# kaushik87599/Melo-GAN

Hardware: AMD Instinct MI355X
Metric: piano-roll samples/sec (G+D step), batch=64 128x256 roll (higher is better)
Workload: dtype f32; 1 GPU; cfg2: 128x256 piano-roll, batch=64 per GPU, full G+D+emotion-D step (1 critic update incl. gradient penalty + 1 generator update); global_batch=64, T=256, C=128, parallelism=dp1, graph=True

## Files before the change

### include/melo_gan_hip.h

```cpp
#ifndef MELO_GAN_HIP_H
#define MELO_GAN_HIP_H

#include <stddef.h>
#include <stdint.h>

#ifdef __cplusplus
extern "C" {
#endif

typedef void* mg_stream_t;

enum { MG_ACT_NONE = 0, MG_ACT_RELU = 1, MG_ACT_LRELU = 2, MG_ACT_GELU = 3, MG_ACT_TANH = 4 };

typedef struct mg_epilogue {
    const float* bias;
    const float* scale;
    const float* shift;
    float* zout;
    int act;
    const float* gref;
    int gact;
    const float* emul;
    const float* gscale;
    int accumulate;
// ... 46 lines not shown
#define MG_CHAIN_SLOTS 6
#define MG_CHAIN_MAX_VEC 512
enum { MG_CH_LOAD = 1, MG_CH_STORE = 2, MG_CH_LAYERNORM = 3, MG_CH_LIN_FWD = 4, MG_CH_LIN_DGRAD = 5, MG_CH_SOFTMAX_CE = 6,
       MG_CH_DHEAD = 7, MG_CH_MEAN_T = 8, MG_CH_COPY = 9 };
typedef struct mg_chain_op {
    int kind;
    int a, b;
    int n0, n1;
    int act;
    int i0, i1;
    float f0;
    const float* p0; long ld0;
    const float* p1; long ld1;
    const float* p2; long ld2;
    const float* p3; long ld3;
    float* q0; long lq0;
    float* q1; long lq1;
    const int64_t* t0;
} mg_chain_op;
int mg_row_chain(const mg_chain_op* ops, int n_ops, int rows, mg_stream_t stream);
int mg_mean_scaled(const float* src, float* out, int n, float scale, mg_stream_t stream);
int mg_stamp(unsigned long long* dst, mg_stream_t stream);

size_t mg_linear_workspace_bytes(int M, int N, int K);
int mg_linear(const float* x, const float* w, float* y, int M, int K, int N, int w_sn, int w_sc,
              const mg_epilogue* epi, int perm_L, void* work, size_t work_bytes, mg_stream_t stream);
int mg_linear_route(int M, int K, int N, int w_sn, int w_sc, int perm_L, int x_aligned, int w_aligned,
                    int* kcontig, int* vec, int* ksplit);

int mg_conv1d_wino3_supported(int B, int T, int Cin, int N);
int mg_wino3_weights(const float* w, float* wt, int N, int Cin, long w_sn, long w_sc, int flip, mg_stream_t stream);
int mg_conv1d_wino3(const float* x, const float* wt, float* y, int B, int T, int Cin, int N, const mg_epilogue* epi,
                    long lds_pad, mg_stream_t stream);
#define MG_MAX_WINO_WJOBS 8
typedef struct mg_wino3_wjob {
    const float* w;
    float* wt;
    int N, Cin;
    long w_sn, w_sc;
    int flip;
} mg_wino3_wjob;
int mg_wino3_weights_multi(const mg_wino3_wjob* jobs, int n_jobs, mg_stream_t stream);

int mg_conv_tile_config(long m_rows, int N, int scatter2);
int mg_conv_plan(int B, int Tm, int Tout, int N, int Cin, int K, int stride, int scatter2, size_t work_bytes,
                 int* ksplit, int* cps);
// ... 253 lines not shown
```

### melo-gan_amd/csrc/common.h

```cpp
#pragma once
#include <hip/hip_runtime.h>
#include <stdio.h>
#include <stdarg.h>
#include <stdint.h>
#include <atomic>
#include "../../include/melo_gan_hip.h"

#define MG_OK 0
#define MG_EARG (-1)
#define MG_EUNSUP (-2)
#define MG_EWORK (-3)
#define MG_EHIP (-4)

void mg_set_error(const char* fmt, ...);

#define MG_CHECK_ARG(cond, ...)                    \
    do {                                           \
        if (!(cond)) {                             \
            mg_set_error(__VA_ARGS__);             \
            return MG_EARG;                        \
        }                                          \
    } while (0)

#define MG_CHECK_LAUNCH(name)                                                   \
    do {                                                                        \
        hipError_t e__ = hipGetLastError();                                     \
        if (e__ != hipSuccess) {                                                \
// ... 191 lines not shown

inline int mg_lds_optin(const void* kernel, std::atomic<uint64_t>& done) {
    int dev = 0;
    MG_HIP(hipGetDevice(&dev));
    const uint64_t bit = dev < 64 ? 1ull << dev : 0;
    if (done.load(std::memory_order_relaxed) & bit) return MG_OK;
    MG_HIP(hipFuncSetAttribute(kernel, hipFuncAttributeMaxDynamicSharedMemorySize, 160 * 1024));
    done.fetch_or(bit, std::memory_order_relaxed);
    return MG_OK;
}

int mg_conv_thin_dispatch(const float* x, const float* w, float* y, int B, int Tin, int Cin, int Tout, int N, int K, int stride,
                          int flip, int transposed, int w_sn, int w_sc, long xbs, long ybs, const mg_epilogue* epi,
                          hipStream_t stream);

int mg_conv_linear_perm(const float* x, const float* w, float* y, int M, int K, int N, int w_sn, const mg_epilogue* epi,
                        int perm_L, hipStream_t stream);

__device__ __forceinline__ int mg_xcd_remap(int id, int n) {
    const int q = n >> 3, r = n & 7, x = id & 7;
    return (x < r ? x * (q + 1) : r * (q + 1) + (x - r) * q) + (id >> 3);
}

static inline int mg_ilog2_ceil(int v) {
    int l = 0;
    while ((1 << l) < v) ++l;
    return l;
}
static inline long mg_cdiv(long a, long b) { return (a + b - 1) / b; }
```

### melo-gan_amd/csrc/linear_skinny.hip

```cpp
#include "common.h"
#include <stdlib.h>
#include <type_traits>

namespace {

struct LinP {
    const float* x;
    const float* w;
    float* y;
    float* part;
    int M, K, N;
    int w_sn, w_sc;
    int ksplit;
    int gx, gy;
    int kw;
    int perm_L, perm_C;
    mg_epilogue e;
};
__device__ __forceinline__ int wrow(const LinP& p, int n) { return p.perm_L ? (n % p.perm_C) * p.perm_L + n / p.perm_C : n; }

constexpr int UNR = 8;
constexpr int NW = 8;

template <bool W_KCONTIG, bool VEC>
__global__ __launch_bounds__(64 * NW) void linear_skinny_kernel(const LinP p) {
    __shared__ float tile[NW][32][33];
    const int tid = threadIdx.x, lane = tid & 63, wave = tid >> 6;
    const int i = lane & 31, h = lane >> 5;
    const int id = mg_xcd_remap((int)blockIdx.x, (int)gridDim.x);
    const int bx = id % p.gx, byz = id / p.gx, by = byz % p.gy, bz = byz / p.gy;
    const int m0 = bx * 32, n0 = by * 32;
    const int row = min(m0 + i, p.M - 1);
    const int col = wrow(p, min(n0 + i, p.N - 1));
// ... 77 lines not shown
    for (int r = 0; r < 16; ++r) tile[wave][(r & 3) + 8 * (r >> 2) + 4 * h][i] = acc[r];
    __syncthreads();
    constexpr int NV = 1024 / (64 * NW);
    float v[NV];
    int nn[NV];
    long di[NV];
    bool ok[NV];
#pragma unroll
    for (int q = 0; q < NV; ++q) {
        const int idx = tid + 64 * NW * q;
        const int rr = idx >> 5, cc = idx & 31;
        const int m = m0 + rr, n = n0 + cc;
        ok[q] = m < p.M && n < p.N;
        nn[q] = ok[q] ? wrow(p, n) : 0;
        di[q] = ok[q] ? (long)m * p.N + n : 0;
        float t = 0.f;
#pragma unroll
        for (int w = 0; w < NW; w += 2) t += tile[w][rr][cc] + tile[w + 1][rr][cc];
        v[q] = t;
    }
    if (p.ksplit > 1) {
#pragma unroll
        for (int q = 0; q < NV; ++q)
            if (ok[q]) p.part[(long)bz * p.M * p.N + di[q]] = v[q];
        return;
    }
    mg_apply_epilogue_set<NV>(p.e, v, nn, di, ok);
#pragma unroll
    for (int q = 0; q < NV; ++q) {
        if (!ok[q]) continue;
        if (p.e.accumulate) v[q] += p.y[di[q]];
        p.y[di[q]] = v[q];
    }
}

__global__ void linear_finish_kernel(const float* __restrict__ part, float* __restrict__ y, long mn, int N, int ksplit,
                                     const mg_epilogue e, int perm_L, int perm_C) {
    const long di = (long)blockIdx.x * blockDim.x + threadIdx.x;
    if (di >= mn) return;
    float v = 0.f;
    for (int z = 0; z < ksplit; ++z) v += part[(long)z * mn + di];
    int n = (int)(di % N);
    if (perm_L) n = (n % perm_C) * perm_L + n / perm_C;
    v = mg_apply_epilogue(e, v, n, di);
    if (e.accumulate) v += y[di];
    y[di] = v;
}

int plan_ksplit(int M, int N, int K) {
    const long tiles = mg_cdiv(M, 32) * mg_cdiv(N, 32);
    int ks = 1;
    while (ks < 32 && K / (NW * ks) > 128 && tiles * ks < 512) ks *= 2;
    return ks;
}

struct LinRoute {
    bool window_gemm;
    bool kcontig, vec;
    int ksplit, kw;
};
LinRoute linear_route(int M, int K, int N, int w_sn, int w_sc, int perm_L, bool x_aligned, bool w_aligned) {
    LinRoute r{};
    if (perm_L > 1 && w_sc == 1 && M >= 128 && (K & 63) == 0 && (N & 63) == 0 && mg_cdiv(M, 64) * (long)(N / 64) >= 192 &&
        x_aligned && w_aligned && (w_sn & 3) == 0 && !getenv("MG_LINEAR_SKINNY_ONLY")) {
        r.window_gemm = true;
        r.ksplit = 1;
        return r;
    }
    r.ksplit = plan_ksplit(M, N, K);
    r.kcontig = (w_sc == 1);
    const int waves = NW * r.ksplit;
    r.vec = (K % (8 * waves) == 0) && x_aligned && (!r.kcontig || (w_aligned && (w_sn & 3) == 0));
    r.kw = r.vec ? K / waves : (int)(mg_cdiv(mg_cdiv(K, waves), 8) * 8);
    return r;
}
bool al16(const void* q) { return (((uintptr_t)q) & 15) == 0; }

}

extern "C" int mg_linear_route(int M, int K, int N, int w_sn, int w_sc, int perm_L, int x_aligned, int w_aligned,
                               int* kcontig, int* vec, int* ksplit) {
    MG_CHECK_ARG(perm_L >= 0 && (perm_L == 0 || N % perm_L == 0), "mg_linear_route: perm_L must divide N");
    MG_CHECK_ARG(M > 0 && K > 0 && N > 0 && w_sn > 0 && w_sc > 0, "mg_linear_route: bad shape");
    MG_CHECK_ARG(w_sn == 1 || w_sc == 1, "mg_linear_route: one weight stride must be 1");
    const LinRoute r = linear_route(M, K, N, w_sn, w_sc, perm_L, x_aligned != 0, w_aligned != 0);
    if (kcontig) *kcontig = r.kcontig;
    if (vec) *vec = r.vec;
    if (ksplit) *ksplit = r.ksplit;
    return r.window_gemm ? 0 : 1;
}

extern "C" size_t mg_linear_workspace_bytes(int M, int N, int K) {
    const int ks = plan_ksplit(M, N, K);
    return ks > 1 ? (size_t)ks * M * N * sizeof(float) : 0;
}

extern "C" int mg_linear(const float* x, const float* w, float* y, int M, int K, int N, int w_sn, int w_sc,
                         const mg_epilogue* epi, int perm_L, void* work, size_t work_bytes, mg_stream_t stream) {
    MG_CHECK_ARG(x && w && y, "mg_linear: null tensor");
    MG_CHECK_ARG(perm_L >= 0 && (perm_L == 0 || N % perm_L == 0), "mg_linear: perm_L must divide N");
    MG_CHECK_ARG(M > 0 && K > 0 && N > 0 && w_sn > 0 && w_sc > 0, "mg_linear: bad shape");
    MG_CHECK_ARG(w_sn == 1 || w_sc == 1, "mg_linear: one weight stride must be 1");
    const LinRoute r = linear_route(M, K, N, w_sn, w_sc, perm_L, al16(x), al16(w));
    if (r.window_gemm)
        return mg_conv_linear_perm(x, w, y, M, K, N, w_sn, epi, perm_L, (hipStream_t)stream);
    LinP p{};
    p.x = x; p.w = w; p.y = y; p.M = M; p.K = K; p.N = N; p.w_sn = w_sn; p.w_sc = w_sc;
    p.e = epi ? *epi : mg_epilogue{};
    p.perm_L = perm_L > 1 ? perm_L : 0;
    p.perm_C = p.perm_L ? N / p.perm_L : 0;
    if (p.e.scale && !p.e.shift) { mg_set_error("mg_linear: scale without shift"); return MG_EARG; }
    p.ksplit = r.ksplit;
    const bool kcontig = r.kcontig, vec = r.vec;
    p.kw = r.kw;
    if (p.ksplit > 1) {
        const size_t need = (size_t)p.ksplit * M * N * sizeof(float);
        if (!work || work_bytes < need) { mg_set_error("mg_linear: workspace too small (%zu < %zu)", work_bytes, need); return MG_EWORK; }
        p.part = (float*)work;
    }
    p.gx = (int)mg_cdiv(M, 32); p.gy = (int)mg_cdiv(N, 32);
    dim3 grid((unsigned)(p.gx * p.gy * p.ksplit));
    hipStream_t st = (hipStream_t)stream;
    if (kcontig) {
        if (vec) hipLaunchKernelGGL((linear_skinny_kernel<true, true>), grid, dim3(64 * NW), 0, st, p);
        else hipLaunchKernelGGL((linear_skinny_kernel<true, false>), grid, dim3(64 * NW), 0, st, p);
    } else {
        if (vec) hipLaunchKernelGGL((linear_skinny_kernel<false, true>), grid, dim3(64 * NW), 0, st, p);
        else hipLaunchKernelGGL((linear_skinny_kernel<false, false>), grid, dim3(64 * NW), 0, st, p);
    }
    MG_CHECK_LAUNCH("linear_skinny_kernel");
    if (p.ksplit > 1) {
        const long mn = (long)M * N;
        hipLaunchKernelGGL(linear_finish_kernel, dim3((unsigned)mg_cdiv(mn, 256)), dim3(256), 0, st,
                           (const float*)work, y, mn, N, p.ksplit, p.e, p.perm_L, p.perm_C);
        MG_CHECK_LAUNCH("linear_finish_kernel");
    }
    return MG_OK;
}
```

### melo-gan_amd/csrc/wgrad_mfma.hip

```cpp
#include "common.h"
#include <stdlib.h>
#include <type_traits>

namespace {

struct WgradP {
    const float* s[2];
    const float* l[2];
    int nb[2];
    float* part;
    float* out;
    float* bias_out;
    int Ts, Tl, A, Bc;
    int tt_log2, n_ttiles;
    int bps;
    int n_bgroups;
    int nbg0;
    long slab;
    long wslab;
    int bias_from;
    int nseg_bias;
    int vec_ok;
    int lin;
    int gx, gy, gz;
};

constexpr int RT = 64;
constexpr int BA = 32, BB = 32;

typedef unsigned u32x4 __attribute__((ext_vector_type(4)));

#ifdef MG_STAMPS
__device__ long long* mg_wstamp_buf = nullptr;
// ... 153 lines not shown
#endif
    MG_STAMP(2);
    float* red = smem;
    float* out = p.part ? p.part + (long)split * p.slab : p.out;
    constexpr int KP = K > 3 ? 3 : K;
    const int nb_cols = min(32, p.Bc - b0);
#pragma unroll
    for (int k0 = 0; k0 < K; k0 += KP) {
        const int kn = (K - k0) < KP ? (K - k0) : KP;
        __syncthreads();
#pragma unroll
        for (int k = k0; k < k0 + kn; ++k)
#pragma unroll
            for (int r = 0; r < 16; ++r)
                red[((wave * KP + (k - k0)) * 32 + (r & 3) + 8 * (r >> 2) + 4 * h) * 33 + (lane & 31)] = acc[k][r];
        __syncthreads();
#pragma unroll 4
        for (int idx = tid; idx < 32 * kn * 32; idx += 256) {
            const int ar = idx / (kn * 32), j = idx - ar * (kn * 32);
            const int bc = j / kn, kk = j - bc * kn;
            const int a = a0 + ar;
            const int o = (kk * 32 + ar) * 33 + bc;
            const float v = (red[o] + red[o + KP * 32 * 33]) + (red[o + 2 * KP * 32 * 33] + red[o + 3 * KP * 32 * 33]);
            if (a < p.A && bc < nb_cols) out[((long)a * p.Bc + b0 + bc) * K + k0 + kk] = v;
        }
    }
    MG_STAMP(3);
}

constexpr int W16_SP = 48;
template <int S> struct W16LP { static constexpr int value = S == 2 ? 40 : 48; };

template <int S, int K>
__device__ __forceinline__ bool wgrad16_applies(const WgradP& p) {
    constexpr int RMAX = (RT - 1) * S + K;
    constexpr int NL4 = (RMAX * (BB / 4) + 255) / 256 + 1;
    const int TT = 1 << p.tt_log2, TB = RT >> p.tt_log2, R = (TT - 1) * S + K;
    return ((p.A & 3) == 0) && ((p.Bc & 3) == 0) && p.vec_ok && (TB * R * (BB / 4) <= 256 * NL4) && p.tt_log2 >= 4;
}

template <int S, int K>
__device__ __forceinline__ void wgrad16_body(const WgradP& p, const int bx, const int by, const int bz) {
    constexpr int PAD = (K - 1) / 2;
    constexpr int RMAX = (RT - 1) * S + K;
    constexpr int NS4 = RT * (BA / 4) / 256;
    constexpr int NL4 = (RMAX * (BB / 4) + 255) / 256 + 1;
    constexpr int SP = W16_SP, LP = W16LP<S>::value;
// ... 131 lines not shown
        for (int k = 0; k < K; ++k) read_b(0, 0, k, fr[0]);
        MG_STAMP(1);
        for (int c = 0;;) {
            chunk(std::integral_constant<int, 0>{}, c);
            if (++c >= n_chunks) break;
            chunk(std::integral_constant<int, 1>{}, c);
            if (++c >= n_chunks) break;
        }
    }
    MG_STAMP(2);

    __syncthreads();
    constexpr int PE = K * 32 + 1;
    float* red = smem;
#pragma unroll
    for (int k = 0; k < K; ++k)
#pragma unroll
        for (int r = 0; r < 4; ++r) red[(16 * wa + 4 * kq + r) * PE + (16 * wb + li) * K + k] = acc[k][r];
    __syncthreads();
    const int nb_valid = min(32, p.Bc - b0) * K;
#pragma unroll 4
    for (int idx = tid; idx < 32 * K * 32; idx += 256) {
        const int ar = idx / (K * 32), j = idx - ar * (K * 32);
        if (a0 + ar < p.A && j < nb_valid) out[((long)(a0 + ar) * p.Bc + b0) * K + j] = red[ar * PE + j];
    }
    MG_STAMP(3);
}

constexpr int LIN_BB = 128;
__device__ __forceinline__ bool wgrad_lin_applies(const WgradP& p) {
    return p.lin != 0;
}
__device__ __forceinline__ void wgrad_lin_body(const WgradP& p, const int bx, const int by, const int bz) {
    extern __shared__ __attribute__((aligned(16))) float smem[];
    constexpr int SPL = 36, LPL = 132;
    float* Ss = smem;
    float* Ls = smem + RT * SPL;
    const int tid = threadIdx.x, lane = tid & 63, wave = tid >> 6, h = lane >> 5, c = lane & 31;
    const int a0 = bx * BA, b0 = by * LIN_BB;
    const int TB = RT;
    const int g_begin = bz * p.bps, g_end = min(g_begin + p.bps, p.n_bgroups);
    f32x16 acc;
#pragma unroll
    for (int i = 0; i < 16; ++i) acc[i] = 0.f;
    for (int g = g_begin; g < g_end; ++g) {
        const int seg_id = g < p.nbg0 ? 0 : 1;
        const int bb0 = (seg_id ? g - p.nbg0 : g) * TB;
// ... 9 lines not shown
            const f32x4 v = *reinterpret_cast<const f32x4*>(Sp + (long)(ok ? r : 0) * p.A + (ok ? a0 + 4 * q : 0));
            *reinterpret_cast<f32x4*>(Ss + r * SPL + 4 * q) = ok ? v : f32x4{0.f, 0.f, 0.f, 0.f};
        }
#pragma unroll
        for (int j = 0; j < 8; ++j) {
            const int idx = tid + 256 * j, r = idx >> 5, q = idx & 31;
            const bool ok = r < rows && b0 + 4 * q < p.Bc;
            const f32x4 v = *reinterpret_cast<const f32x4*>(Lp + (long)(ok ? r : 0) * p.Bc + (ok ? b0 + 4 * q : 0));
            *reinterpret_cast<f32x4*>(Ls + r * LPL + 4 * q) = ok ? v : f32x4{0.f, 0.f, 0.f, 0.f};
        }
        __syncthreads();
#pragma unroll 8
        for (int r2 = 0; r2 < RT / 2; ++r2) {
            const int r = 2 * r2 + h;
            acc = __builtin_amdgcn_mfma_f32_32x32x2f32(Ss[r * SPL + c], Ls[r * LPL + 32 * wave + c], acc, 0, 0, 0);
        }
    }
    float* out = p.part ? p.part + (long)bz * p.slab : p.out;
    const int b = b0 + 32 * wave + c;
    if (b < p.Bc) {
#pragma unroll
        for (int i = 0; i < 16; ++i) {
            const int a = a0 + (i & 3) + 8 * (i >> 2) + 4 * h;
            if (a < p.A) out[(long)a * p.Bc + b] = acc[i];
        }
    }
}

__device__ __forceinline__ void wgrad_bias_body(const WgradP& p, const int cb, const int bz) {
    extern __shared__ __attribute__((aligned(16))) float smem[];
    f32x4* bred = reinterpret_cast<f32x4*>(smem);
    const int tid = threadIdx.x, q = tid & 7, rl = tid >> 3;
    const bool from_s = p.bias_from == 1;
    const int C = from_s ? p.A : p.Bc, T = from_s ? p.Ts : p.Tl;
    const int TB = RT >> p.tt_log2;
    const int g_begin = bz * p.bps, g_end = min(g_begin + p.bps, p.n_bgroups);
    f32x4 acc = {0.f, 0.f, 0.f, 0.f};
    const int c = cb * 32 + 4 * q;
    for (int seg = 0; seg < p.nseg_bias && seg < 2; ++seg) {
        const int gs = seg ? p.nbg0 : 0, ge = seg ? p.n_bgroups : p.nbg0;
        const int ga = max(g_begin, gs), gb = min(g_end, ge);
        if (ga >= gb) continue;
        const int b_lo = (ga - gs) * TB, b_hi = min((gb - gs) * TB, p.nb[seg]);
        const float* base = (from_s ? p.s[seg] : p.l[seg]) + (long)b_lo * T * C;
        const long rows = (long)(b_hi - b_lo) * T;
        if (c + 3 < C && (C & 3) == 0 && p.vec_ok) {
            long r = rl;
            for (; r + 32 * 7 < rows; r += 32 * 8) {
                f32x4 v[8];
#pragma unroll
                for (int u = 0; u < 8; ++u) v[u] = *reinterpret_cast<const f32x4*>(base + (r + 32 * u) * C + c);
#pragma unroll
                for (int u = 0; u < 8; ++u) acc += v[u];
            }
            for (; r < rows; r += 32) acc += *reinterpret_cast<const f32x4*>(base + r * C + c);
        } else {
            for (long r = rl; r < rows; r += 32)
#pragma unroll
                for (int e = 0; e < 4; ++e)
                    if (c + e < C) acc[e] += base[r * C + c + e];
        }
    }
    bred[tid] = acc;
    __syncthreads();
    if (tid < 32) {
        const int ch = cb * 32 + tid;
        if (ch < C) {
            float v = 0.f;
#pragma unroll 8
            for (int g = 0; g < 32; ++g) v += bred[8 * g + (tid >> 2)][tid & 3];
            if (p.part) p.part[(long)bz * p.slab + p.wslab + ch] = v;
            else p.bias_out[ch] = v;
        }
    }
}

struct WgradJobs {
    WgradP p[MG_MAX_WGRAD_JOBS];
    int first[MG_MAX_WGRAD_JOBS + 1];
    int bfirst[MG_MAX_WGRAD_JOBS + 1];
    int n;
};
template <int S, int K>
__global__ __launch_bounds__(256, 2) void wgrad_multi_kernel(const WgradJobs J) {
    const int bid = (int)blockIdx.x;
    const bool tile = bid < J.first[J.n];
    const int* first = tile ? J.first : J.bfirst;
    int j = 0;
    while (j + 1 < J.n && bid >= first[j + 1]) ++j;
    const int b = bid - first[j];
    const WgradP& p = J.p[j];
    if (tile) {
        const int gxy = p.gx * p.gy, bz = b / gxy, r = b - bz * gxy;
        if (K == 1 && wgrad_lin_applies(p)) wgrad_lin_body(p, r % p.gx, r / p.gx, bz);
        else if (wgrad16_applies<S, K>(p)) wgrad16_body<S, K>(p, r % p.gx, r / p.gx, bz);
        else wgrad_body<S, K>(p, r % p.gx, r / p.gx, bz);
    } else {
        const int ncb = ((p.bias_from == 1 ? p.A : p.Bc) + 31) >> 5;
        wgrad_bias_body(p, b % ncb, b / ncb);
    }
}

struct ReduceJobs {
    const float* part[MG_MAX_WGRAD_JOBS];
    float* out[MG_MAX_WGRAD_JOBS];
    float* bias_out[MG_MAX_WGRAD_JOBS];
    long n[MG_MAX_WGRAD_JOBS], wn[MG_MAX_WGRAD_JOBS];
    int nsplit[MG_MAX_WGRAD_JOBS];
    int first[MG_MAX_WGRAD_JOBS + 1];
    int njobs;
};
__global__ __launch_bounds__(256) void reduce_slabs_multi_kernel(const ReduceJobs J) {
    __shared__ float sh[4][64];
    int j = 0;
    while (j + 1 < J.njobs && (int)blockIdx.x >= J.first[j + 1]) ++j;
    const float* __restrict__ part = J.part[j];
    const long n = J.n[j], wn = J.wn[j];
    const int nsplit = J.nsplit[j];
    const int ex = threadIdx.x & 63, g = threadIdx.x >> 6;
    const long i = (long)((int)blockIdx.x - J.first[j]) * 64 + ex;
    float s = 0.f;
    if (i < n)
// ... 34 lines not shown
    if (want > ngroups) want = ngroups;
    if (want > MAX_SPLITS) want = MAX_SPLITS;
    if (want < 1) want = 1;
    pl.bps = (int)mg_cdiv(ngroups, want);
    pl.nsplit = (int)mg_cdiv(ngroups, pl.bps);
    return pl;
}

}

#ifdef MG_STAMPS
extern "C" int mg_dbg_set_wstamps(long long* buf) {
    return hipMemcpyToSymbol(HIP_SYMBOL(mg_wstamp_buf), &buf, sizeof(buf)) == hipSuccess ? 0 : 1;
}
#endif

extern "C" size_t mg_wgrad_workspace_bytes(int A, int Bc, int K, int nb_total, int Ts) {
    int lg = mg_ilog2_ceil(Ts);
    const int lgrt = mg_ilog2_ceil(RT);
    if (lg > lgrt) lg = lgrt;
    const int TB = RT >> lg;
    long ns = mg_cdiv(nb_total, TB) + 1;
    if (ns > MAX_SPLITS) ns = MAX_SPLITS;
    return (size_t)ns * ((size_t)A * (size_t)Bc * (size_t)K + (size_t)(A > Bc ? A : Bc)) * sizeof(float);
}

namespace {
int build_wgrad(const float* s0, const float* l0, int nb0, const float* s1, const float* l1, int nb1, float* out,
                float* bias_out, int bias_from, int Ts, int Tl, int A, int Bc, int K, int stride, void* work,
                size_t work_bytes, WgradP& p, Plan& pl, size_t& lds, dim3& grid, long want_slices = 0) {
    MG_CHECK_ARG(bias_from >= 0 && bias_from <= 2 && ((bias_from == 0) == (bias_out == nullptr)),
                 "mg_wgrad: bias_out and bias_from (1: sums of S, 2: sums of L) must be given together");
    MG_CHECK_ARG(s0 && l0 && out && nb0 > 0, "mg_wgrad: null/empty segment 0");
    MG_CHECK_ARG(nb1 == 0 || (s1 && l1), "mg_wgrad: null segment 1");
    MG_CHECK_ARG(Ts > 0 && Tl > 0 && A > 0 && Bc > 0, "mg_wgrad: bad shape");
    MG_CHECK_ARG(K == 1 || K == 3 || K == 5, "mg_wgrad: K=%d unsupported", K);
    MG_CHECK_ARG(stride == 1 || stride == 2, "mg_wgrad: stride=%d unsupported", stride);
    if (stride == 2 && K != 5) {
        mg_set_error("mg_wgrad: stride 2 needs K=5");
        return MG_EUNSUP;
    }
    pl = make_plan(A, Bc, K, nb0, nb1, Ts, want_slices);
    const long wslab = (long)A * Bc * K;
    const long slab = wslab + (bias_from == 1 ? A : bias_from == 2 ? Bc : 0);
    if (pl.nsplit > 1 && (!work || work_bytes < (size_t)pl.nsplit * slab * sizeof(float))) {
        mg_set_error("mg_wgrad: workspace too small (%zu < %zu)", work_bytes, (size_t)pl.nsplit * slab * sizeof(float));
        return MG_EWORK;
// ... 41 lines not shown
    return MG_OK;
}
}

extern "C" int mg_wgrad_multi(const mg_wgrad_job* jobs, int n_jobs, int K, int stride, void* work, size_t work_bytes,
                              mg_stream_t stream);

extern "C" int mg_wgrad(const float* s0, const float* l0, int nb0, const float* s1, const float* l1, int nb1,
                        float* out, float* bias_out, int bias_from, int Ts, int Tl, int A, int Bc, int K, int stride,
                        void* work, size_t work_bytes, mg_stream_t stream) {
    mg_wgrad_job j{};
    j.s0 = s0; j.l0 = l0; j.nb0 = nb0;
    j.s1 = s1; j.l1 = l1; j.nb1 = nb1;
    j.out = out; j.bias_out = bias_out; j.bias_from = bias_from;
    j.Ts = Ts; j.Tl = Tl; j.A = A; j.Bc = Bc;
    return mg_wgrad_multi(&j, 1, K, stride, work, work_bytes, stream);
}

extern "C" int mg_wgrad_multi(const mg_wgrad_job* jobs, int n_jobs, int K, int stride, void* work, size_t work_bytes,
                              mg_stream_t stream) {
    MG_CHECK_ARG(jobs && n_jobs > 0 && n_jobs <= MG_MAX_WGRAD_JOBS, "mg_wgrad_multi: 1..%d jobs", MG_MAX_WGRAD_JOBS);
    WgradJobs J{};
    ReduceJobs Rj{};
    size_t lds_max = 0, used = 0;
    int nblocks = 0, rblocks = 0;
    long want[MG_MAX_WGRAD_JOBS];
    {
        long target = 512;
        if (const char* f = getenv("MG_WGRAD_TARGET")) target = atol(f);
        long tiles[MG_MAX_WGRAD_JOBS], chunks[MG_MAX_WGRAD_JOBS], total = 0;
        for (int i = 0; i < n_jobs; ++i) {
            const mg_wgrad_job& q = jobs[i];
            MG_CHECK_ARG(q.A > 0 && q.Bc > 0 && q.Ts > 0 && q.Tl > 0 && q.nb0 > 0 && q.nb1 >= 0 && q.s0 && q.l0 && q.out,
                         "mg_wgrad_multi: job %d: null/empty segment 0 or bad shape", i);
            const Plan pl = make_plan(q.A, q.Bc, K, q.nb0, q.nb1, q.Ts);
            tiles[i] = mg_cdiv(q.A, BA) * mg_cdiv(q.Bc, BB);
            chunks[i] = (long)(pl.nbg0 + pl.nbg1) * pl.n_ttiles;
            total += tiles[i] * chunks[i];
        }
        long cpw = mg_cdiv(total, target);
        for (int it = 0; it < 64; ++it) {
            long wgs = 0;
            for (int i = 0; i < n_jobs; ++i) {
                const mg_wgrad_job& q = jobs[i];
                want[i] = (chunks[i] + cpw / 2) / cpw;
                if (want[i] < 1) want[i] = 1;
                const Plan pl = make_plan(q.A, q.Bc, K, q.nb0, q.nb1, q.Ts, want[i]);
                wgs += tiles[i] * pl.nsplit;
            }
            if (wgs <= target) break;
            cpw += mg_cdiv(cpw, 16);
        }
    }
    for (int i = 0; i < n_jobs; ++i) {
        const mg_wgrad_job& q = jobs[i];
        Plan pl;
        size_t lds;
        dim3 grid;
        const size_t need = mg_wgrad_workspace_bytes(q.A, q.Bc, K, q.nb0 + q.nb1, q.Ts);
        void* w = used < work_bytes && work ? (char*)work + used : nullptr;
        const int rc = build_wgrad(q.s0, q.l0, q.nb0, q.s1, q.l1, q.nb1, q.out, q.bias_out, q.bias_from, q.Ts, q.Tl, q.A,
                                   q.Bc, K, stride, w, w ? work_bytes - used : 0, J.p[i], pl, lds, grid, want[i]);
        if (rc != MG_OK) return rc;
        if (pl.nsplit > 1) {
            used += (need + 255) & ~(size_t)255;
            const int r = Rj.njobs++;
            Rj.part[r] = J.p[i].part; Rj.out[r] = q.out; Rj.bias_out[r] = q.bias_out;
            Rj.n[r] = J.p[i].slab; Rj.wn[r] = J.p[i].wslab; Rj.nsplit[r] = pl.nsplit;
            Rj.first[r] = rblocks;
            rblocks += (int)mg_cdiv(J.p[i].slab, 64);
        }
        lds_max = lds > lds_max ? lds : lds_max;
        const int ntile = J.p[i].gx * J.p[i].gy * J.p[i].gz;
        J.first[i] = nblocks;
        nblocks += ntile;
        J.bfirst[i] = (int)grid.x - ntile;
    }
    J.first[n_jobs] = nblocks;
    for (int i = 0; i < n_jobs; ++i) {
        const int nb = J.bfirst[i];
        J.bfirst[i] = nblocks;
        nblocks += nb;
    }
    J.bfirst[n_jobs] = nblocks;
    J.n = n_jobs;
    Rj.first[Rj.njobs] = rblocks;
    hipStream_t st = (hipStream_t)stream;
#define MG_WG(S_, K_) hipLaunchKernelGGL((wgrad_multi_kernel<S_, K_>), dim3((unsigned)nblocks), dim3(256), lds_max, st, J)
    if (stride == 1) {
        if (K == 1) MG_WG(1, 1); else if (K == 3) MG_WG(1, 3); else MG_WG(1, 5);
    } else {
        MG_WG(2, 5);
    }
#undef MG_WG
    MG_CHECK_LAUNCH("wgrad_multi_kernel");
    if (Rj.njobs > 0) {
        hipLaunchKernelGGL(reduce_slabs_multi_kernel, dim3((unsigned)rblocks), dim3(256), 0, st, Rj);
        MG_CHECK_LAUNCH("reduce_slabs_multi_kernel");
    }
    return MG_OK;
}
```

### melo-gan_amd/ops.py

```python
from __future__ import annotations

import ctypes as C
import functools
import math
from typing import Optional

import torch

from . import _lib as L
from ._lib import ACT_NONE, ACT_RELU, ACT_LRELU, ACT_GELU, ACT_TANH, Epilogue

Tensor = torch.Tensor


def _stream() -> C.c_void_p:
    return C.c_void_p(torch.cuda.current_stream().cuda_stream)


def _p(t: Optional[Tensor]):
    return None if t is None else C.c_void_p(t.data_ptr())


def _chk(t: Tensor, name: str, shape=None, dtype=torch.float32):
    if not isinstance(t, torch.Tensor) or not t.is_cuda:
# ... 326 lines not shown
    L.check(rc, "mg_conv16")
    return y


SKINNY_MAX_ROWS = 512


def linear_route(M: int, K: int, N: int, w_sn: int, w_sc: int, perm_L: int = 0, x_aligned: bool = True, w_aligned: bool = True):
    lib = L.load()
    kc, vec, ks = C.c_int(), C.c_int(), C.c_int()
    rc = lib.mg_linear_route(M, K, N, w_sn, w_sc, perm_L, int(x_aligned), int(w_aligned), C.byref(kc), C.byref(vec), C.byref(ks))
    if rc < 0:
        L.check(rc, "mg_linear_route")
    if rc == 0:
        return "conv_wgemm_kernel<1,1,false,true,%s>" % {22: "2,2", 12: "1,2", 11: "1,1"}[lib.mg_conv_tile_config(M, N, 0)], 1
    return "linear_skinny_kernel<%s,%s>" % ("true" if kc.value else "false", "true" if vec.value else "false"), ks.value


def _linear(x, w, y, K, N, w_sn, w_sc, epi, perm_L=0):
    M = x.shape[0]
    e = epilogue((M, N), N, **epi)
    lib = L.load()
    need = lib.mg_linear_workspace_bytes(M, N, K)
    work = workspace(need, x.device, "linear") if need else None
    sym = lambda: linear_route(M, K, N, w_sn, w_sc, perm_L, x.data_ptr() % 16 == 0, w.data_ptr() % 16 == 0)[0]
    with _observe(sym, 2.0 * M * N * K):
        rc = lib.mg_linear(_p(x), _p(w), _p(y), M, K, N, w_sn, w_sc, C.byref(e), perm_L, _p(work),
                           work.numel() if work is not None else 0, _stream())
    L.check(rc, "mg_linear")
    return y


def linear_fwd(x, w, y, perm_L: int = 0, **epi):
    _chk(x, "x")
    _chk(w, "w")
    _chk(y, "y")
    out_f, in_f = w.shape
    B = x.shape[0]
    if perm_L:
        if B > SKINNY_MAX_ROWS or out_f % perm_L or x.dim() != 2 or x.shape[1] != in_f or tuple(y.shape) != (B, perm_L, out_f // perm_L):
            raise ValueError(f"linear_fwd(perm_L={perm_L}): shape mismatch x{tuple(x.shape)} w{tuple(w.shape)} y{tuple(y.shape)}")
        return _linear(x, w, y, in_f, out_f, in_f, 1, epi, perm_L)
    if x.dim() != 2 or x.shape[1] != in_f or tuple(y.shape) != (B, out_f):
        raise ValueError(f"linear_fwd: shape mismatch x{tuple(x.shape)} w{tuple(w.shape)} y{tuple(y.shape)}")
    if B <= SKINNY_MAX_ROWS:
        return _linear(x, w, y, in_f, out_f, in_f, 1, epi)
    conv_gather(x.view(B, 1, in_f), w, y.view(B, 1, out_f), out_f, 1, 1, in_f, 1, **epi)
# ... 205 lines not shown
            _chk(ly["dw"], "dw", tuple(w.shape))
            a.dw = ly["dw"].data_ptr()
    return arr


def spectral_norm_fwd(layers, train: bool, eps: float = 1e-12):
    arr = _sn_jobs(layers, False)
    L.check(L.load().mg_spectral_norm_fwd(arr, len(layers), 1 if train else 0, float(eps), _stream()), "mg_spectral_norm_fwd")


def spectral_norm_bwd(layers):
    arr = _sn_jobs(layers, True)
    L.check(L.load().mg_spectral_norm_bwd(arr, len(layers), _stream()), "mg_spectral_norm_bwd")


def stamp(buf, i: int):
    L.check(L.load().mg_stamp(buf.data_ptr() + 8 * int(i), _stream()), "mg_stamp")


_ws_cache = {}
_ws_retired = []


def workspace(nbytes: int, device, tag: str = "default") -> Tensor:
    key = (str(device), tag, torch.cuda.current_stream().cuda_stream)
    buf = _ws_cache.get(key)
    if buf is None or buf.numel() < nbytes:
        if buf is not None:
            _ws_retired.append(buf)
        size = max(nbytes, 1 << 20, 2 * buf.numel() if buf is not None else 0)
        buf = torch.empty(size, dtype=torch.uint8, device=device)
        _ws_cache[key] = buf
    return buf


def wgrad(small: Tensor, large: Tensor, out: Tensor, K: int, stride: int,
          small2: Optional[Tensor] = None, large2: Optional[Tensor] = None, work: Optional[Tensor] = None,
          bias_out: Optional[Tensor] = None, bias_from: int = 0):
    _chk(small, "small")
    _chk(large, "large")
    _chk(out, "out")
    nb0, Ts, A = small.shape
    if large.shape[0] != nb0:
        raise ValueError("wgrad: batch mismatch")
    Tl, Bc = large.shape[1], large.shape[2]
    pad = (K - 1) // 2
    if (Tl + 2 * pad - K) // stride + 1 != Ts and not (stride == 2 and Tl == 2 * Ts):
        raise ValueError(f"wgrad: Ts={Ts} inconsistent with Tl={Tl}, K={K}, stride={stride}")
    if out.numel() != A * Bc * K:
        raise ValueError(f"wgrad: out numel {out.numel()} != {A * Bc * K}")
    nb1 = 0
    if small2 is not None:
        _chk(small2, "small2")
        _chk(large2, "large2")
        nb1 = small2.shape[0]
        if tuple(small2.shape[1:]) != (Ts, A) or tuple(large2.shape) != (nb1, Tl, Bc):
            raise ValueError("wgrad: segment 1 shape mismatch")
    if bias_out is not None:
        _chk(bias_out, "bias_out", (A if bias_from == 1 else Bc,))
        if bias_from not in (1, 2):
            raise ValueError("wgrad: bias_from must be 1 (S) or 2 (L) when bias_out is given")
    elif bias_from:
        raise ValueError("wgrad: bias_from without bias_out")
    lib = L.load()
    need = lib.mg_wgrad_workspace_bytes(A, Bc, K, nb0 + nb1, Ts)
    if work is None:
        work = workspace(need, small.device, "wgrad")
    if work.numel() * work.element_size() < need:
        raise ValueError("wgrad: workspace too small")
    with _observe(lambda: f"wgrad_multi_kernel<{stride},{K}>", 2.0 * (nb0 + nb1) * Ts * A * Bc * K):
        rc = lib.mg_wgrad(_p(small), _p(large), nb0, _p(small2), _p(large2), nb1, _p(out), _p(bias_out), bias_from,
                          Ts, Tl, A, Bc, K, stride, _p(work), work.numel() * work.element_size(), _stream())
    L.check(rc, "mg_wgrad")
    return out


def _wgrad_job(small, large, out, K, stride, small2=None, large2=None, bias_out=None, bias_from=0):
    _chk(small, "small")
    _chk(large, "large")
    _chk(out, "out")
    nb0, Ts, A = small.shape
    Tl, Bc = large.shape[1], large.shape[2]
    pad = (K - 1) // 2
    if large.shape[0] != nb0 or ((Tl + 2 * pad - K) // stride + 1 != Ts and not (stride == 2 and Tl == 2 * Ts)):
        raise ValueError(f"wgrad: S {tuple(small.shape)} inconsistent with L {tuple(large.shape)}, K={K}, stride={stride}")
    if out.numel() != A * Bc * K:
        raise ValueError(f"wgrad: out numel {out.numel()} != {A * Bc * K}")
    nb1 = 0
    if small2 is not None:
        _chk(small2, "small2")
# ... 7 lines not shown
        _chk(bias_out, "bias_out", (A if bias_from == 1 else Bc,))
    elif bias_from:
        raise ValueError("wgrad: bias_from without bias_out")
    return (small, large, nb0, small2, large2, nb1, out, bias_out, bias_from, Ts, Tl, A, Bc, K, stride)


def wgrad_multi(jobs, tag=""):
    lib = L.load()
    groups = {}
    for j in jobs:
        groups.setdefault((j[13], j[14]), []).append(j)
    for (K, stride), js in groups.items():
        for i in range(0, len(js), L.MAX_WGRAD_JOBS):
            part = js[i:i + L.MAX_WGRAD_JOBS]
            arr = (L.WgradJob * len(part))()
            need, flops = 0, 0.0
            for a, (s0, l0, nb0, s1, l1, nb1, out, bo, bf, Ts, Tl, A, Bc, _, _) in zip(arr, part):
                a.s0, a.l0, a.nb0 = s0.data_ptr(), l0.data_ptr(), nb0
                a.s1, a.l1, a.nb1 = (None if s1 is None else s1.data_ptr()), (None if l1 is None else l1.data_ptr()), nb1
                a.out, a.bias_out, a.bias_from = out.data_ptr(), (None if bo is None else bo.data_ptr()), bf
                a.Ts, a.Tl, a.A, a.Bc = Ts, Tl, A, Bc
                need += (lib.mg_wgrad_workspace_bytes(A, Bc, K, nb0 + nb1, Ts) + 255) & ~255
                flops += 2.0 * (nb0 + nb1) * Ts * A * Bc * K
            work = workspace(need, part[0][0].device, "wgrad_multi" + tag)
            with _observe(lambda: f"wgrad_multi_kernel<{stride},{K}>", flops):
                rc = lib.mg_wgrad_multi(arr, len(part), K, stride, _p(work), work.numel() * work.element_size(), _stream())
            L.check(rc, "mg_wgrad_multi")


def conv1d_wgrad(x, dy, dw, stride, x2=None, dy2=None, db=None, defer=False):
    K = dw.shape[2]
    if defer:
        return _wgrad_job(dy, x, dw, K, stride, dy2, x2, db, 1 if db is not None else 0)
    return wgrad(dy, x, dw, K, stride, dy2, x2, bias_out=db, bias_from=1 if db is not None else 0)


def convT1d_wgrad(x, dy, dw, db=None, defer=False):
    if defer:
        return _wgrad_job(x, dy, dw, 5, 2, None, None, db, 2 if db is not None else 0)
    return wgrad(x, dy, dw, 5, 2, bias_out=db, bias_from=2 if db is not None else 0)


def linear_wgrad(x, dy, dw, x2=None, dy2=None, db=None, defer=False):
    B = x.shape[0]
    s2 = l2 = None
    if x2 is not None:
        s2, l2 = dy2.view(dy2.shape[0], 1, -1), x2.view(x2.shape[0], 1, -1)
# ... 1368 lines not shown
```

Before: 78530 samples/s.

## Fuse split-K reductions into producer kernels via last-block atomic counters

Split-K linear and weight-gradient kernels now write partial slabs with agent-scope stores and bump a per-tile atomic counter. The last block to arrive sums all slabs and applies the epilogue, so the separate finish and reduce kernel launches are no longer needed. This removes one launch and one dependency per split-K op. In exchange, the last block does a serial reduction, counters live in zeroed workspace, and correctness depends on the fence and counter-reset logic.

```diff
diff --git a/include/melo_gan_hip.h b/include/melo_gan_hip.h
--- a/include/melo_gan_hip.h
+++ b/include/melo_gan_hip.h
@@ -92,6 +92,7 @@
 int mg_mean_scaled(const float* src, float* out, int n, float scale, mg_stream_t stream);
 int mg_stamp(unsigned long long* dst, mg_stream_t stream);
 
+#define MG_SPLITK_COUNTER_BYTES 16384
 size_t mg_linear_workspace_bytes(int M, int N, int K);
 int mg_linear(const float* x, const float* w, float* y, int M, int K, int N, int w_sn, int w_sc,
               const mg_epilogue* epi, int perm_L, void* work, size_t work_bytes, mg_stream_t stream);
diff --git a/melo-gan_amd/csrc/common.h b/melo-gan_amd/csrc/common.h
--- a/melo-gan_amd/csrc/common.h
+++ b/melo-gan_amd/csrc/common.h
@@ -3,6 +3,8 @@
 #include <stdio.h>
 #include <stdarg.h>
 #include <stdint.h>
+#include <stdlib.h>
+#include <string.h>
 #include <atomic>
 #include "../../include/melo_gan_hip.h"
 
@@ -240,6 +242,30 @@
     return (x < r ? x * (q + 1) : r * (q + 1) + (x - r) * q) + (id >> 3);
 }
 
+constexpr int MG_SPLITK_COUNTERS = MG_SPLITK_COUNTER_BYTES / 4;
+__device__ __forceinline__ void mg_slab_store(float* p, float v, bool wt) {
+    if (wt) __hip_atomic_store(p, v, __ATOMIC_RELAXED, __HIP_MEMORY_SCOPE_AGENT);
+    else *p = v;
+}
+__device__ __forceinline__ bool mg_splitk_last(unsigned* counter, int nsplit, unsigned* lds_word) {
+    __builtin_amdgcn_s_waitcnt(0x0F70);
+    __syncthreads();
+    if (threadIdx.x == 0) *lds_word = atomicAdd(counter, 1u);
+    __syncthreads();
+    if (*lds_word != (unsigned)(nsplit - 1)) return false;
+    __builtin_amdgcn_fence(__ATOMIC_ACQUIRE, "agent");
+    if (threadIdx.x == 0) __hip_atomic_store(counter, 0u, __ATOMIC_RELAXED, __HIP_MEMORY_SCOPE_AGENT);
+    return true;
+}
+inline bool mg_splitk_two_launch(const char* family, bool family_default) {
+    const char* f = getenv("MG_SPLITK_TWO_LAUNCH");
+    if (!f || !*f) return family_default;
+    if (!strcmp(f, "0")) return false;
+    if (!strcmp(f, "1")) return true;
+    if (!strcmp(f, "linear") || !strcmp(f, "wgrad")) return !strcmp(f, family);
+    return family_default;
+}
+
 static inline int mg_ilog2_ceil(int v) {
     int l = 0;
     while ((1 << l) < v) ++l;
diff --git a/melo-gan_amd/csrc/linear_skinny.hip b/melo-gan_amd/csrc/linear_skinny.hip
--- a/melo-gan_amd/csrc/linear_skinny.hip
+++ b/melo-gan_amd/csrc/linear_skinny.hip
@@ -9,6 +9,7 @@
     const float* w;
     float* y;
     float* part;
+    unsigned* cnt;
     int M, K, N;
     int w_sn, w_sc;
     int ksplit;
@@ -132,7 +133,23 @@
     if (p.ksplit > 1) {
 #pragma unroll
         for (int q = 0; q < NV; ++q)
-            if (ok[q]) p.part[(long)bz * p.M * p.N + di[q]] = v[q];
+            if (ok[q]) mg_slab_store(p.part + (long)bz * p.M * p.N + di[q], v[q], p.cnt != nullptr);
+        if (!p.cnt) return;
+        if (!mg_splitk_last(p.cnt + by * p.gx + bx, p.ksplit, reinterpret_cast<unsigned*>(&tile[0][0][0]))) return;
+        const long mn = (long)p.M * p.N;
+#pragma unroll
+        for (int q = 0; q < NV; ++q) v[q] = 0.f;
+#pragma unroll 4
+        for (int z = 0; z < p.ksplit; ++z)
+#pragma unroll
+            for (int q = 0; q < NV; ++q) v[q] += p.part[(long)z * mn + di[q]];
+#pragma unroll
+        for (int q = 0; q < NV; ++q) {
+            if (!ok[q]) continue;
+            float t = mg_apply_epilogue(p.e, v[q], nn[q], di[q]);
+            if (p.e.accumulate) t += p.y[di[q]];
+            p.y[di[q]] = t;
+        }
         return;
     }
     mg_apply_epilogue_set<NV>(p.e, v, nn, di, ok);
@@ -161,6 +178,11 @@
     const long tiles = mg_cdiv(M, 32) * mg_cdiv(N, 32);
     int ks = 1;
     while (ks < 32 && K / (NW * ks) > 128 && tiles * ks < 512) ks *= 2;
+    if (ks > 1)
+        if (const char* f = getenv("MG_LINEAR_KSPLIT")) {
+            const int v = atoi(f);
+            if (v >= 2 && v <= 32 && (v & (v - 1)) == 0 && K / (NW * v) >= 8) ks = v;
+        }
     return ks;
 }
 
@@ -202,7 +224,7 @@
 
 extern "C" size_t mg_linear_workspace_bytes(int M, int N, int K) {
     const int ks = plan_ksplit(M, N, K);
-    return ks > 1 ? (size_t)ks * M * N * sizeof(float) : 0;
+    return ks > 1 ? MG_SPLITK_COUNTER_BYTES + (size_t)ks * M * N * sizeof(float) : 0;
 }
 
 extern "C" int mg_linear(const float* x, const float* w, float* y, int M, int K, int N, int w_sn, int w_sc,
@@ -224,11 +246,12 @@
     const bool kcontig = r.kcontig, vec = r.vec;
     p.kw = r.kw;
     if (p.ksplit > 1) {
-        const size_t need = (size_t)p.ksplit * M * N * sizeof(float);
+        const size_t need = MG_SPLITK_COUNTER_BYTES + (size_t)p.ksplit * M * N * sizeof(float);
         if (!work || work_bytes < need) { mg_set_error("mg_linear: workspace too small (%zu < %zu)", work_bytes, need); return MG_EWORK; }
-        p.part = (float*)work;
+        p.part = (float*)((char*)work + MG_SPLITK_COUNTER_BYTES);
     }
     p.gx = (int)mg_cdiv(M, 32); p.gy = (int)mg_cdiv(N, 32);
+    if (p.ksplit > 1 && p.gx * p.gy <= MG_SPLITK_COUNTERS && !mg_splitk_two_launch("linear", true)) p.cnt = (unsigned*)work;
     dim3 grid((unsigned)(p.gx * p.gy * p.ksplit));
     hipStream_t st = (hipStream_t)stream;
     if (kcontig) {
@@ -239,10 +262,10 @@
         else hipLaunchKernelGGL((linear_skinny_kernel<false, false>), grid, dim3(64 * NW), 0, st, p);
     }
     MG_CHECK_LAUNCH("linear_skinny_kernel");
-    if (p.ksplit > 1) {
+    if (p.ksplit > 1 && !p.cnt) {
         const long mn = (long)M * N;
         hipLaunchKernelGGL(linear_finish_kernel, dim3((unsigned)mg_cdiv(mn, 256)), dim3(256), 0, st,
-                           (const float*)work, y, mn, N, p.ksplit, p.e, p.perm_L, p.perm_C);
+                           (const float*)p.part, y, mn, N, p.ksplit, p.e, p.perm_L, p.perm_C);
         MG_CHECK_LAUNCH("linear_finish_kernel");
     }
     return MG_OK;
diff --git a/melo-gan_amd/csrc/wgrad_mfma.hip b/melo-gan_amd/csrc/wgrad_mfma.hip
--- a/melo-gan_amd/csrc/wgrad_mfma.hip
+++ b/melo-gan_amd/csrc/wgrad_mfma.hip
@@ -9,6 +9,7 @@
     const float* l[2];
     int nb[2];
     float* part;
+    unsigned* cnt;
     float* out;
     float* bias_out;
     int Ts, Tl, A, Bc;
@@ -208,7 +209,7 @@
             const int a = a0 + ar;
             const int o = (kk * 32 + ar) * 33 + bc;
             const float v = (red[o] + red[o + KP * 32 * 33]) + (red[o + 2 * KP * 32 * 33] + red[o + 3 * KP * 32 * 33]);
-            if (a < p.A && bc < nb_cols) out[((long)a * p.Bc + b0 + bc) * K + k0 + kk] = v;
+            if (a < p.A && bc < nb_cols) mg_slab_store(out + ((long)a * p.Bc + b0 + bc) * K + k0 + kk, v, p.cnt != nullptr);
         }
     }
     MG_STAMP(3);
@@ -386,7 +387,7 @@
 #pragma unroll 4
     for (int idx = tid; idx < 32 * K * 32; idx += 256) {
         const int ar = idx / (K * 32), j = idx - ar * (K * 32);
-        if (a0 + ar < p.A && j < nb_valid) out[((long)(a0 + ar) * p.Bc + b0) * K + j] = red[ar * PE + j];
+        if (a0 + ar < p.A && j < nb_valid) mg_slab_store(out + ((long)(a0 + ar) * p.Bc + b0) * K + j, red[ar * PE + j], p.cnt != nullptr);
     }
     MG_STAMP(3);
 }
@@ -442,7 +443,7 @@
 #pragma unroll
         for (int i = 0; i < 16; ++i) {
             const int a = a0 + (i & 3) + 8 * (i >> 2) + 4 * h;
-            if (a < p.A) out[(long)a * p.Bc + b] = acc[i];
+            if (a < p.A) mg_slab_store(out + (long)a * p.Bc + b, acc[i], p.cnt != nullptr);
         }
     }
 }
@@ -489,10 +490,40 @@
             float v = 0.f;
 #pragma unroll 8
             for (int g = 0; g < 32; ++g) v += bred[8 * g + (tid >> 2)][tid & 3];
-            if (p.part) p.part[(long)bz * p.slab + p.wslab + ch] = v;
+            if (p.part) mg_slab_store(p.part + (long)bz * p.slab + p.wslab + ch, v, p.cnt != nullptr);
             else p.bias_out[ch] = v;
         }
     }
+}
+
+__device__ __forceinline__ float wgrad_slab_sum(const float* part, long slab, int nsplit, long i) {
+    float s[4] = {0.f, 0.f, 0.f, 0.f};
+#pragma unroll 2
+    for (int z0 = 0; z0 < nsplit; z0 += 4)
+#pragma unroll
+        for (int g = 0; g < 4; ++g)
+            if (z0 + g < nsplit) s[g] += part[(long)(z0 + g) * slab + i];
+    return (s[0] + s[1]) + (s[2] + s[3]);
+}
+template <int K>
+__device__ __forceinline__ void wgrad_finish_tile(const WgradP& p, const int bx, const int by) {
+    extern __shared__ __attribute__((aligned(16))) float smem[];
+    if (!mg_splitk_last(p.cnt + by * p.gx + bx, p.gz, reinterpret_cast<unsigned*>(smem))) return;
+    const int bbt = p.lin ? LIN_BB : BB;
+    const int a0 = bx * BA, b0 = by * bbt;
+    const int rows = min(BA, p.A - a0), w = min(bbt, p.Bc - b0) * K;
+    for (int idx = threadIdx.x; idx < rows * w; idx += 256) {
+        const int ar = idx / w, j = idx - ar * w;
+        const long i = ((long)(a0 + ar) * p.Bc + b0) * K + j;
+        p.out[i] = wgrad_slab_sum(p.part, p.slab, p.gz, i);
+    }
+}
+__device__ __forceinline__ void wgrad_finish_bias(const WgradP& p, const int cb) {
+    extern __shared__ __attribute__((aligned(16))) float smem[];
+    if (!mg_splitk_last(p.cnt + p.gx * p.gy + cb, p.gz, reinterpret_cast<unsigned*>(smem))) return;
+    const int C = p.bias_from == 1 ? p.A : p.Bc;
+    const int ch = cb * 32 + (int)threadIdx.x;
+    if (threadIdx.x < 32 && ch < C) p.bias_out[ch] = wgrad_slab_sum(p.part, p.slab, p.gz, p.wslab + ch);
 }
 
 struct WgradJobs {
@@ -515,9 +546,11 @@
         if (K == 1 && wgrad_lin_applies(p)) wgrad_lin_body(p, r % p.gx, r / p.gx, bz);
         else if (wgrad16_applies<S, K>(p)) wgrad16_body<S, K>(p, r % p.gx, r / p.gx, bz);
         else wgrad_body<S, K>(p, r % p.gx, r / p.gx, bz);
+        if (p.cnt) wgrad_finish_tile<K>(p, r % p.gx, r / p.gx);
     } else {
         const int ncb = ((p.bias_from == 1 ? p.A : p.Bc) + 31) >> 5;
         wgrad_bias_body(p, b % ncb, b / ncb);
+        if (p.cnt) wgrad_finish_bias(p, b % ncb);
     }
 }
 
@@ -598,7 +631,7 @@
     const int TB = RT >> lg;
     long ns = mg_cdiv(nb_total, TB) + 1;
     if (ns > MAX_SPLITS) ns = MAX_SPLITS;
-    return (size_t)ns * ((size_t)A * (size_t)Bc * (size_t)K + (size_t)(A > Bc ? A : Bc)) * sizeof(float);
+    return MG_SPLITK_COUNTER_BYTES + (size_t)ns * ((size_t)A * (size_t)Bc * (size_t)K + (size_t)(A > Bc ? A : Bc)) * sizeof(float);
 }
 
 namespace {
@@ -686,8 +719,8 @@
     MG_CHECK_ARG(jobs && n_jobs > 0 && n_jobs <= MG_MAX_WGRAD_JOBS, "mg_wgrad_multi: 1..%d jobs", MG_MAX_WGRAD_JOBS);
     WgradJobs J{};
     ReduceJobs Rj{};
-    size_t lds_max = 0, used = 0;
-    int nblocks = 0, rblocks = 0;
+    size_t lds_max = 0, used = MG_SPLITK_COUNTER_BYTES;
+    int nblocks = 0, rblocks = 0, ncnt = 0;
     long want[MG_MAX_WGRAD_JOBS];
     {
         long target = 512;
@@ -721,7 +754,7 @@
         Plan pl;
         size_t lds;
         dim3 grid;
-        const size_t need = mg_wgrad_workspace_bytes(q.A, q.Bc, K, q.nb0 + q.nb1, q.Ts);
+        const size_t need = mg_wgrad_workspace_bytes(q.A, q.Bc, K, q.nb0 + q.nb1, q.Ts) - MG_SPLITK_COUNTER_BYTES;
         void* w = used < work_bytes && work ? (char*)work + used : nullptr;
         const int rc = build_wgrad(q.s0, q.l0, q.nb0, q.s1, q.l1, q.nb1, q.out, q.bias_out, q.bias_from, q.Ts, q.Tl, q.A,
                                    q.Bc, K, stride, w, w ? work_bytes - used : 0, J.p[i], pl, lds, grid, want[i]);
@@ -733,6 +766,8 @@
             Rj.n[r] = J.p[i].slab; Rj.wn[r] = J.p[i].wslab; Rj.nsplit[r] = pl.nsplit;
             Rj.first[r] = rblocks;
             rblocks += (int)mg_cdiv(J.p[i].slab, 64);
+            J.p[i].cnt = (unsigned*)work + ncnt;
+            ncnt += J.p[i].gx * J.p[i].gy + (q.bias_from ? (int)mg_cdiv(q.bias_from == 1 ? q.A : q.Bc, 32) : 0);
         }
         lds_max = lds > lds_max ? lds : lds_max;
         const int ntile = J.p[i].gx * J.p[i].gy * J.p[i].gz;
@@ -749,6 +784,9 @@
     J.bfirst[n_jobs] = nblocks;
     J.n = n_jobs;
     Rj.first[Rj.njobs] = rblocks;
+    const bool in_launch = Rj.njobs > 0 && ncnt <= MG_SPLITK_COUNTERS && !mg_splitk_two_launch("wgrad", true);
+    if (!in_launch)
+        for (int i = 0; i < n_jobs; ++i) J.p[i].cnt = nullptr;
     hipStream_t st = (hipStream_t)stream;
 #define MG_WG(S_, K_) hipLaunchKernelGGL((wgrad_multi_kernel<S_, K_>), dim3((unsigned)nblocks), dim3(256), lds_max, st, J)
     if (stride == 1) {
@@ -758,7 +796,7 @@
     }
 #undef MG_WG
     MG_CHECK_LAUNCH("wgrad_multi_kernel");
-    if (Rj.njobs > 0) {
+    if (Rj.njobs > 0 && !in_launch) {
         hipLaunchKernelGGL(reduce_slabs_multi_kernel, dim3((unsigned)rblocks), dim3(256), 0, st, Rj);
         MG_CHECK_LAUNCH("reduce_slabs_multi_kernel");
     }
diff --git a/melo-gan_amd/ops.py b/melo-gan_amd/ops.py
--- a/melo-gan_amd/ops.py
+++ b/melo-gan_amd/ops.py
@@ -372,7 +372,7 @@
     e = epilogue((M, N), N, **epi)
     lib = L.load()
     need = lib.mg_linear_workspace_bytes(M, N, K)
-    work = workspace(need, x.device, "linear") if need else None
+    work = workspace(need, x.device, "linear", zeroed=True) if need else None
     sym = lambda: linear_route(M, K, N, w_sn, w_sc, perm_L, x.data_ptr() % 16 == 0, w.data_ptr() % 16 == 0)[0]
     with _observe(sym, 2.0 * M * N * K):
         rc = lib.mg_linear(_p(x), _p(w), _p(y), M, K, N, w_sn, w_sc, C.byref(e), perm_L, _p(work),
@@ -624,14 +624,14 @@
 _ws_retired = []
 
 
-def workspace(nbytes: int, device, tag: str = "default") -> Tensor:
+def workspace(nbytes: int, device, tag: str = "default", zeroed: bool = False) -> Tensor:
     key = (str(device), tag, torch.cuda.current_stream().cuda_stream)
     buf = _ws_cache.get(key)
     if buf is None or buf.numel() < nbytes:
         if buf is not None:
             _ws_retired.append(buf)
         size = max(nbytes, 1 << 20, 2 * buf.numel() if buf is not None else 0)
-        buf = torch.empty(size, dtype=torch.uint8, device=device)
+        buf = (torch.zeros if zeroed else torch.empty)(size, dtype=torch.uint8, device=device)
         _ws_cache[key] = buf
     return buf
 
@@ -667,7 +667,7 @@
     lib = L.load()
     need = lib.mg_wgrad_workspace_bytes(A, Bc, K, nb0 + nb1, Ts)
     if work is None:
-        work = workspace(need, small.device, "wgrad")
+        work = workspace(need, small.device, "wgrad", zeroed=True)
     if work.numel() * work.element_size() < need:
         raise ValueError("wgrad: workspace too small")
     with _observe(lambda: f"wgrad_multi_kernel<{stride},{K}>", 2.0 * (nb0 + nb1) * Ts * A * Bc * K):
@@ -721,7 +721,7 @@
                 a.Ts, a.Tl, a.A, a.Bc = Ts, Tl, A, Bc
                 need += (lib.mg_wgrad_workspace_bytes(A, Bc, K, nb0 + nb1, Ts) + 255) & ~255
                 flops += 2.0 * (nb0 + nb1) * Ts * A * Bc * K
-            work = workspace(need, part[0][0].device, "wgrad_multi" + tag)
+            work = workspace(need, part[0][0].device, "wgrad_multi" + tag, zeroed=True)
             with _observe(lambda: f"wgrad_multi_kernel<{stride},{K}>", flops):
                 rc = lib.mg_wgrad_multi(arr, len(part), K, stride, _p(work), work.numel() * work.element_size(), _stream())
             L.check(rc, "mg_wgrad_multi")
```

Measured after the change: 78320 samples/s. Within noise of the previous version (-0.3%).
